# andrewcharlesjones/spatial-alignment

Measured on AMD Instinct MI355X. Metric: training steps/sec (ELBO fwd+bwd), 2-view N=10k M=200, 1/2/4/8 GPU, higher is better.
Workload: dtype f32 (fp64 warp layer, covariance whitening and M x M factorisations)

## Files before the change

### spatial_alignment_amd/csrc/qf_common.hpp

```cpp
#pragma once
#include <stdlib.h>

#include "common.hpp"

namespace gpsa {

typedef float f32x4_t __attribute__((ext_vector_type(4)));

typedef float f32x4 __attribute__((ext_vector_type(4)));
typedef float f32x2 __attribute__((ext_vector_type(2)));

enum { MODE_QUAD = 0, MODE_ACCUM = 1, MODE_STORE = 2 };

enum { PACK_SYM_UPPER = 1, PACK_KSTEP = 2, PACK_KSTEP_LAST = 4 };

typedef __attribute__((address_space(3))) void* lds_ptr_t;

__device__ __forceinline__ void glds16(const float* gsrc, unsigned lds_base) {
  unsigned keep;
  asm volatile(
      "s_mov_b32 %0, m0\n\ts_mov_b32 m0, %2\n\ts_nop 0\n\tglobal_load_lds_dwordx4 %1, off\n\ts_mov_b32 m0, %0"
      : "=&s"(keep)
      : "v"(gsrc), "s"(lds_base)
      : "memory");
}
__device__ __forceinline__ void dma_set_m0(unsigned lds_base) {
  asm volatile("s_mov_b32 m0, %0\n\ts_nop 0" ::"s"(lds_base) : "memory");
}
template <int IMM>
__device__ __forceinline__ void glds16_m0(const float* gsrc_minus_imm) {
  static_assert(IMM >= 0 && IMM < 4096, "immediate offset of a global instruction");
  asm volatile("global_load_lds_dwordx4 %0, off offset:%1" ::"v"(gsrc_minus_imm), "n"(IMM) : "memory");
}
template <int IMM>
__device__ __forceinline__ void glds4_m0(const float* gsrc_minus_imm) {
  static_assert(IMM >= 0 && IMM < 4096, "immediate offset of a global instruction");
  asm volatile("global_load_lds_dword %0, off offset:%1" ::"v"(gsrc_minus_imm), "n"(IMM) : "memory");
}
#define GPSA_DMA_DRAIN() asm volatile("s_waitcnt vmcnt(0)" ::: "memory")
#define GPSA_DMA_WAIT(N) asm volatile("s_waitcnt vmcnt(%0)" ::"n"(N) : "memory")
__device__ __forceinline__ unsigned lds_addr(const void* p) {
  return (unsigned)(unsigned long long)(lds_ptr_t)(p);
}

#define GPSA_PANEL_MAX_C (1LL << 26)
template <int MB, int NCT, bool QO, bool FULLT = false>
__device__ __forceinline__ void load_alpha_slab(const float* __restrict__ X, int M, long long C, long long cw, int j,
                                                int kq, float (&xb)[NCT][MB][4], bool (&okc)[NCT]) {
  const int Mm1 = M - 1;
  const unsigned Cu = (unsigned)C;
#pragma unroll
  for (int ct = 0; ct < NCT; ++ct) {
    const long long c = cw + ct * 16 + j;
    okc[ct] = c < C;
    const unsigned cl = (unsigned)(okc[ct] ? c : C - 1);
#pragma unroll
    for (int t = 0; t < MB; ++t)
#pragma unroll
      for (int r = 0; r < 4; ++r) {
        const int want = t * 16 + (QO ? r : r * 4);
        const int lane_row = QO ? kq * 4 : kq;
        if (FULLT && t < MB - 1) {
          xb[ct][t][r] = (X + (long long)want * C)[(unsigned)lane_row * Cu + cl];
        } else {
          const int bu = want < Mm1 ? want : Mm1;
          const int lp = lane_row < Mm1 - bu ? lane_row : Mm1 - bu;
          xb[ct][t][r] = (X + (long long)bu * C)[(unsigned)lp * Cu + cl];
        }
      }
  }
#pragma unroll
  for (int ct = 0; ct < NCT; ++ct)
#pragma unroll
    for (int t = 0; t < MB; ++t)
#pragma unroll
      for (int r = 0; r < 4; ++r)
        xb[ct][t][r] = (okc[ct] && t * 16 + (QO ? kq * 4 + r : r * 4 + kq) < M) ? xb[ct][t][r] : 0.f;
}
template <int MB, int NCT, int NR>
__device__ __forceinline__ void load_alpha_last(const float* __restrict__ X, int M, long long C, long long cw, int j,
                                                int kq, int nlive, float (&xl)[NCT][NR]) {
#pragma unroll
  for (int ct = 0; ct < NCT; ++ct) {
    const long long c = cw + ct * 16 + j;
    const bool ok = c < C;
    const float* __restrict__ Xc = X + (ok ? c : C - 1);
    float v[NR];
#pragma unroll
    for (int r = 0; r < NR; ++r) {
      const int row = (MB - 1) * 16 + r * 4 + kq;
      v[r] = Xc[(long long)(row < M ? row : M - 1) * C];
    }
#pragma unroll
    for (int r = 0; r < NR; ++r) xl[ct][r] = (r < nlive && ok && (MB - 1) * 16 + r * 4 + kq < M) ? v[r] : 0.f;
  }
}

struct TileOrder {
  long long tile0, tile1, nfull, n;
  int lo0, hi1, L, fp, lp;
  __device__ TileOrder(long long it0, long long it1, int L_) {
    L = L_;
    tile0 = it0 / L;
    tile1 = (it1 - 1) / L;
    lo0 = (int)(it0 - tile0 * L);
    hi1 = (int)(it1 - 1 - tile1 * L);
    if (tile0 == tile1) {
      fp = lp = 0;
      nfull = 0;
      n = 1;
    } else {
      fp = lo0 != 0;
      lp = hi1 != L - 1;
      nfull = (tile1 - lp) - (tile0 + fp) + 1;
      n = nfull + fp + lp;
    }
  }
  __device__ void get(long long step, long long& tile, int& a, int& b) const {
    if (tile0 == tile1) {
      tile = tile0; a = lo0; b = hi1;
    } else if (step < nfull) {
      tile = tile0 + fp + step; a = 0; b = L - 1;
    } else if (lp && step == nfull) {
      tile = tile1; a = 0; b = hi1;
    } else {
      tile = tile0; a = lo0; b = L - 1;
    }
  }
};

struct GramBigArgs {
  const float* alpha;
  const float* g;
  float* part;
  int M, L, nsplit, nblk;
  long long C, Cpad;
  int lb;
};
__global__ void pad_rows_kernel(const float* __restrict__ g, int L, long long C, long long Cpad,
                                float* __restrict__ gpad);
void gram_big_launch(dim3 grid, hipStream_t st, const GramBigArgs& a);
struct ProdBigArgs {
  const float* P;
  const float* X;
  float* W;
  int M, Mp, L;
  long long C;
};
__global__ void __launch_bounds__(256, 2) prod_big_kernel(ProdBigArgs a);
template <typename TO>
__global__ void __launch_bounds__(256) gram_big_reduce_kernel(const float* __restrict__ part, int M, int nsplit, TO* __restrict__ out);
static inline int big_remap_lb() { return 16; }

struct BigQuadArgs {
  const float* P;
  const float* X;
  float* v;
  float* W;
  int M, Mp, L;
  long long C;
  int lb;
};

struct BigAccumArgs {
  const float* P;
  const float* X;
  const float* g;
  float* out;
  int M, Mp, L, nrb, nsplit;
  long long C, ctiles;
  float scale;
};

__global__ void __launch_bounds__(256) big_accum_reduce_kernel(const float* __restrict__ part, int nsplit, long long n4, float* __restrict__ out);
static inline bool big_panel_ok(int M, long long C, int L, const void* alpha) {
  return M > 128 && (C & 3) == 0 && C >= 128 && cdiv(C, 128) * cdiv(M, 128) * 32 < 0x7fffffffLL && L <= 65535 &&
         (reinterpret_cast<uintptr_t>(alpha) & 15) == 0;
}
static inline int big_accum_nsplit(int M, long long C, int L) {
  const long long wgs = cdiv(M, 128) * cdiv(C, 128), slots = 2LL * num_cus();
  int best = 1;
  double beff = 0.0;
  for (int s = 1; s <= 4 && (s == 1 || L / s >= 8); ++s) {
    const double eff = (double)(wgs * s) / (double)(cdiv(wgs * s, slots) * slots);
    if (eff > beff) { beff = eff; best = s; }
    if (eff >= 0.9) break;
  }
  return best;
}
static inline long long big_accum_ws_bytes(int M, long long C, int L) {
  const int ns = big_accum_nsplit(M, C, L);
  return ns > 1 ? (long long)ns * M * C * 4 : 0;
}

template <typename TS>
__global__ void pad_k_kernel(const TS* __restrict__ src, int M, int Mp, long long n, float* __restrict__ dst);
template <typename TS>
__global__ void pad_k_tri_kernel(const TS* __restrict__ src, int M, int Mp, long long n, float* __restrict__ dst);
template <bool TRI, bool STORE, int NS>
__global__ void __launch_bounds__(256, 2) big_quad_kernel(BigQuadArgs a);
template <int NS>
__global__ void __launch_bounds__(256, 2) big_accum_kernel(BigAccumArgs a);
extern template __global__ void pad_k_kernel<float>(const float* __restrict__, int, int, long long, float* __restrict__);
extern template __global__ void pad_k_kernel<double>(const double* __restrict__, int, int, long long, float* __restrict__);
extern template __global__ void pad_k_tri_kernel<float>(const float* __restrict__, int, int, long long, float* __restrict__);
extern template __global__ void pad_k_tri_kernel<double>(const double* __restrict__, int, int, long long, float* __restrict__);
extern template __global__ void big_quad_kernel<true, false, 3>(BigQuadArgs);
extern template __global__ void big_quad_kernel<false, true, 3>(BigQuadArgs);
extern template __global__ void big_accum_kernel<3>(BigAccumArgs);
extern template __global__ void gram_big_reduce_kernel<float>(const float* __restrict__, int, int, float* __restrict__);

constexpr int panel_wgs_per_cu(int MB, int NCT) { return (MB * NCT >= 24) ? 1 : 2; }
constexpr int elbo_wgs_per_cu(int MB, int NCT) { return (MB * NCT >= 14) ? 1 : 2; }
#define GPSA_SHAPE_SECOND(MB, SECOND, ...) \
  if (mb == MB) return SECOND;

template <int MB, int NCT, int MODE, int RL>
__global__ void __launch_bounds__(256, panel_wgs_per_cu(MB, NCT)) panel_mfma_kernel(const float* __restrict__ Ppk, const float* __restrict__ X, const float* __restrict__ g, int M, long long C, int L, float* __restrict__ out, float* __restrict__ colsq, float out_scale, float* __restrict__ slab, float* __restrict__ keep);
#define GPSA_PANEL_SIG (const float* __restrict__ Ppk, const float* __restrict__ X, const float* __restrict__ g, int M, long long C, int L, float* __restrict__ out, float* __restrict__ colsq, float out_scale, float* __restrict__ slab, float* __restrict__ keep)
#define GPSA_PANEL_SHAPES(X, MODE) X(2, 4, MODE) X(4, 4, MODE) X(7, 4, MODE) X(13, 3, MODE) X(16, 2, MODE)
#define GPSA_PANEL_SHAPES_BIG(X, MODE) X(24, 1, MODE) X(32, 1, MODE)
#define GPSA_PANEL_EXTERN(MB, NCT, MODE)                                              \
  extern template __global__ void panel_mfma_kernel<MB, NCT, MODE, 2> GPSA_PANEL_SIG; \
  extern template __global__ void panel_mfma_kernel<MB, NCT, MODE, 4> GPSA_PANEL_SIG;
#define GPSA_PANEL_DEFINE(MB, NCT, MODE)                                       \
  template __global__ void panel_mfma_kernel<MB, NCT, MODE, 2> GPSA_PANEL_SIG; \
  template __global__ void panel_mfma_kernel<MB, NCT, MODE, 4> GPSA_PANEL_SIG;
GPSA_PANEL_SHAPES(GPSA_PANEL_EXTERN, MODE_QUAD)
GPSA_PANEL_SHAPES(GPSA_PANEL_EXTERN, MODE_STORE)
GPSA_PANEL_SHAPES(GPSA_PANEL_EXTERN, MODE_ACCUM)
GPSA_PANEL_SHAPES_BIG(GPSA_PANEL_EXTERN, MODE_ACCUM)
constexpr int panel_nct_for(int mb) {
  GPSA_PANEL_SHAPES(GPSA_SHAPE_SECOND, 0)
  GPSA_PANEL_SHAPES_BIG(GPSA_SHAPE_SECOND, 0)
  return 0;
}

struct ElboArgs {
  const float* Ppk;
  const float* X;
  int M;
  long long C;
  int L;
  const float* meanT;
  const double* q;
  const float* var_u;
  const float* eps;
  const float* Y;
  const float* noise_u;
  long long N;
  int S;
  float* g;
  float* dmeanT;
  float* FT;
  float* abar;
  float* slab;
  double* part;
  int nparts;
};

template <int MB, int NCT, int RL, bool FULLT = false, bool PAIRB = false>
__global__ void __launch_bounds__(256, elbo_wgs_per_cu(MB, NCT)) panel_elbo_kernel(ElboArgs a);
#define GPSA_ELBO_SHAPES(X) X(2, 4) X(4, 4) X(7, 4) X(13, 2) X(16, 2)
#define GPSA_ELBO_EXTERN(MB, NCT)                                          \
  extern template __global__ void panel_elbo_kernel<MB, NCT, 2>(ElboArgs); \
  extern template __global__ void panel_elbo_kernel<MB, NCT, 4>(ElboArgs);
#define GPSA_ELBO_DEFINE(MB, NCT)                                   \
  template __global__ void panel_elbo_kernel<MB, NCT, 2>(ElboArgs); \
  template __global__ void panel_elbo_kernel<MB, NCT, 4>(ElboArgs);
GPSA_ELBO_SHAPES(GPSA_ELBO_EXTERN)
constexpr int elbo_nct_for(int mb) {
  GPSA_ELBO_SHAPES(GPSA_SHAPE_SECOND)
  return 0;
}
extern template __global__ void panel_elbo_kernel<13, 2, 2, true, true>(ElboArgs);
extern template __global__ void panel_elbo_kernel<13, 2, 4, true, true>(ElboArgs);
template <int MB, int NCT, int RL, bool FULLT = false, bool PAIRB = false>
__global__ void __launch_bounds__(256, elbo_wgs_per_cu(MB, NCT)) panel_elbo_skip_kernel(ElboArgs a);
#define GPSA_ELBO_SKIP_EXTERN(MB, NCT)                                          \
  extern template __global__ void panel_elbo_skip_kernel<MB, NCT, 2>(ElboArgs); \
  extern template __global__ void panel_elbo_skip_kernel<MB, NCT, 4>(ElboArgs);
#define GPSA_ELBO_SKIP_DEFINE(MB, NCT)                                   \
  template __global__ void panel_elbo_skip_kernel<MB, NCT, 2>(ElboArgs); \
  template __global__ void panel_elbo_skip_kernel<MB, NCT, 4>(ElboArgs);
GPSA_ELBO_SHAPES(GPSA_ELBO_SKIP_EXTERN)
extern template __global__ void panel_elbo_skip_kernel<13, 2, 2, true, true>(ElboArgs);
extern template __global__ void panel_elbo_skip_kernel<13, 2, 4, true, true>(ElboArgs);
template <int MB, int NCT, int RL, bool FULLT = false, bool PAIRB = false>
__global__ void __launch_bounds__(256, elbo_wgs_per_cu(MB, NCT))
panel_elbo_pois_kernel(ElboArgs a, const float* __restrict__ log_offset, int skip);
#define GPSA_ELBO_POIS_EXTERN(MB, NCT)                                                              \
  extern template __global__ void panel_elbo_pois_kernel<MB, NCT, 2>(ElboArgs, const float*, int); \
  extern template __global__ void panel_elbo_pois_kernel<MB, NCT, 4>(ElboArgs, const float*, int);
#define GPSA_ELBO_POIS_DEFINE(MB, NCT)                                                       \
  template __global__ void panel_elbo_pois_kernel<MB, NCT, 2>(ElboArgs, const float*, int); \
  template __global__ void panel_elbo_pois_kernel<MB, NCT, 4>(ElboArgs, const float*, int);
GPSA_ELBO_SHAPES(GPSA_ELBO_POIS_EXTERN)
extern template __global__ void panel_elbo_pois_kernel<13, 2, 2, true, true>(ElboArgs, const float*, int);
extern template __global__ void panel_elbo_pois_kernel<13, 2, 4, true, true>(ElboArgs, const float*, int);

template <int MB, int NCT>
__global__ void __launch_bounds__(256, 1) panel_elbo_x3_kernel(ElboArgs a);
#define GPSA_ELBO_X3_SHAPES(X) X(2, 2) X(4, 2) X(7, 2) X(13, 1) X(16, 1)
#define GPSA_ELBO_X3_EXTERN(MB, NCT) extern template __global__ void panel_elbo_x3_kernel<MB, NCT>(ElboArgs);
#define GPSA_ELBO_X3_DEFINE(MB, NCT) template __global__ void panel_elbo_x3_kernel<MB, NCT>(ElboArgs);
GPSA_ELBO_X3_SHAPES(GPSA_ELBO_X3_EXTERN)
constexpr int elbo_x3_nct_for(int mb) {
  GPSA_ELBO_X3_SHAPES(GPSA_SHAPE_SECOND)
  return 0;
}
template <typename TS>
__global__ void __launch_bounds__(256) pack_x3_kernel(const TS* __restrict__ src, int M, int MB, int KB, int L,
                                                       unsigned short* __restrict__ dst, const float* __restrict__ drow);
extern template __global__ void pack_x3_kernel<float>(const float* __restrict__, int, int, int, int,
                                                      unsigned short* __restrict__, const float* __restrict__);
extern template __global__ void pack_x3_kernel<double>(const double* __restrict__, int, int, int, int,
                                                       unsigned short* __restrict__, const float* __restrict__);

template <int MB, int NCT, int RL>
__global__ void __launch_bounds__(256, panel_wgs_per_cu(MB, NCT)) quad_sym_mfma_kernel(const float* __restrict__ Ppk, const float* __restrict__ X, int M, long long C, int L, float* __restrict__ out);
#define GPSA_SYM_SIG (const float* __restrict__ Ppk, const float* __restrict__ X, int M, long long C, int L, float* __restrict__ out)
#define GPSA_SYM_SHAPES(X) X(2, 4) X(4, 4) X(7, 4) X(13, 3) X(16, 2) X(24, 1)
#define GPSA_SYM_EXTERN(MB, NCT)                                                 \
  extern template __global__ void quad_sym_mfma_kernel<MB, NCT, 2> GPSA_SYM_SIG; \
  extern template __global__ void quad_sym_mfma_kernel<MB, NCT, 4> GPSA_SYM_SIG;
#define GPSA_SYM_DEFINE(MB, NCT)                                          \
  template __global__ void quad_sym_mfma_kernel<MB, NCT, 2> GPSA_SYM_SIG; \
  template __global__ void quad_sym_mfma_kernel<MB, NCT, 4> GPSA_SYM_SIG;
GPSA_SYM_SHAPES(GPSA_SYM_EXTERN)

constexpr int GR_KC = 64;
template <int MB, bool ALIGNED, int NL>
__global__ void __launch_bounds__(256, (MB >= 13 || NL > 1) ? 1 : 2) gram_mfma_kernel(const float* __restrict__ alpha, const float* __restrict__ g, long long gstride, int M, long long C, int L, int nsplit, float* __restrict__ part, const float* __restrict__ dmean);
#define GPSA_GRAM_SIG (const float* __restrict__ alpha, const float* __restrict__ g, long long gstride, int M, long long C, int L, int nsplit, float* __restrict__ part, const float* __restrict__ dmean)
template <int MB>
struct GramPlan {
  static constexpr int NT = MB * (MB + 1) / 2;
  int cnt[4];
  int rr[4][NT], cc[4][NT];
  constexpr GramPlan() : cnt{}, rr{}, cc{} {
    const int cap = (NT + 3) / 4;
    for (int r = MB - 1; r >= 0; --r) {
      int best = -1;
      for (int w = 0; w < 4 && best < 0; ++w)
        if (cnt[w] + r + 1 <= cap) best = w;
      if (best < 0) {
        best = 0;
        for (int w = 1; w < 4; ++w)
          if (cnt[w] < cnt[best]) best = w;
      }
      for (int c = 0; c <= r; ++c) {
        rr[best][cnt[best]] = r;
        cc[best][cnt[best]] = c;
        ++cnt[best];
      }
    }
  }
  constexpr int max_cnt() const {
    int m = 0;
    for (int w = 0; w < 4; ++w) m = cnt[w] > m ? cnt[w] : m;
    return m;
  }
};

#define GPSA_GRAM_SHAPES(X) X(2, 2) X(4, 2) X(7, 2) X(13, 2) X(2, 1) X(4, 1) X(7, 1) X(13, 1) X(16, 1)
#define GPSA_GRAM_EXTERN(MB, NL)                                                \
  extern template __global__ void gram_mfma_kernel<MB, true, NL> GPSA_GRAM_SIG; \
  extern template __global__ void gram_mfma_kernel<MB, false, NL> GPSA_GRAM_SIG;
#define GPSA_GRAM_DEFINE(MB, NL)                                         \
  template __global__ void gram_mfma_kernel<MB, true, NL> GPSA_GRAM_SIG; \
  template __global__ void gram_mfma_kernel<MB, false, NL> GPSA_GRAM_SIG;
GPSA_GRAM_SHAPES(GPSA_GRAM_EXTERN)
constexpr int gram_max_nl(int mb) {
  GPSA_GRAM_SHAPES(GPSA_SHAPE_SECOND)
  return 0;
}
template <typename TO>
__global__ void gram_reduce_kernel(const float* __restrict__ part, int M, int MP, int L, int nsplit, TO* __restrict__ out,
                                   float* __restrict__ ddelta, float dbeta);
extern template __global__ void gram_reduce_kernel<float>(const float* __restrict__, int, int, int, int, float* __restrict__, float* __restrict__, float);
extern template __global__ void gram_reduce_kernel<double>(const float* __restrict__, int, int, int, int, double* __restrict__, float* __restrict__, float);

template <int MB>
__global__ void __launch_bounds__(256, 1) gram_x3_kernel(const unsigned short* __restrict__ img, const float* __restrict__ g,
                                                         const float* __restrict__ dmean, int M, long long C, int L,
                                                         int nsplit, float* __restrict__ part);
#define GPSA_GRAM_X3_SHAPES(X) X(2) X(4) X(7) X(13) X(16)
#define GPSA_GRAM_X3_EXTERN(MB)                                                                                          \
  extern template __global__ void gram_x3_kernel<MB>(const unsigned short* __restrict__, const float* __restrict__,       \
                                                     const float* __restrict__, int, long long, int, int, float* __restrict__);
GPSA_GRAM_X3_SHAPES(GPSA_GRAM_X3_EXTERN)
__global__ void __launch_bounds__(256) split_image_kernel(const float* __restrict__ X, int M, int MB, long long C, long long KBc,
                                                          unsigned short* __restrict__ dst);

}
```

### spatial_alignment_amd/csrc/qf_gram.hip

```cpp
#include "qf_common.hpp"

namespace gpsa {

__device__ __attribute__((aligned(16))) const float gram_zero16[4] = {0.f, 0.f, 0.f, 0.f};


constexpr int GR_G = 4;

template <int MB, int NKB, int W, int NS, int NL, typename STG>
__device__ __forceinline__ void gram_wave_chunk(const float* __restrict__ img,
                                                const float* __restrict__ gvec, int kq,
                                                f32x4 (&acc)[NL][NS + GR_G], STG&& stage, int drow, int lane15) {
  constexpr GramPlan<MB> P{};
  constexpr int N = P.cnt[W];
  constexpr int NGRP = (((NS + GR_G - 1) / GR_G) + 1) & ~1;
  constexpr int NPW_ = (MB * NKB + 3) / 4;
  static_assert(NKB == 4, "one K block per staging wave");
  auto frag = [&](int kb, int tile_row) {
    return *reinterpret_cast<const float4*>(img + kb * (NPW_ * 256) + tile_row * 256);
  };
  auto tile_of = [](int s) { return s < N ? s : N - 1; };
  auto new_row = [&](int s) { return s < N && (s == 0 || P.rr[W][s] != P.rr[W][s - 1]); };
  float4 araw[2][GR_G], fb[2][GR_G];
  float4 gk[NL], gn[NL], arow[NL];
#pragma unroll
  for (int q = 0; q < NL; ++q) {
    gn[q] = gk[q] = *reinterpret_cast<const float4*>(gvec + q * GR_KC + kq * 4);
    arow[q] = make_float4(0.f, 0.f, 0.f, 0.f);
  }
  constexpr bool OWNS_LAST = [] {
    constexpr GramPlan<MB> Q{};
    for (int s = 0; s < Q.cnt[W]; ++s)
      if (Q.rr[W][s] == MB - 1) return true;
    return false;
  }();
  const bool dsel = OWNS_LAST && drow >= 0 && lane15 == drow;
  float4 dk[OWNS_LAST ? NL : 1], dn[OWNS_LAST ? NL : 1];
  if (OWNS_LAST) {
#pragma unroll
    for (int q = 0; q < NL; ++q)
      dn[q] = dk[q] = drow >= 0 ? *reinterpret_cast<const float4*>(gvec + (NL + q) * GR_KC + kq * 4)
                                : make_float4(0.f, 0.f, 0.f, 0.f);
  }
#define GPSA_GR_FETCH(SLOT, KB, GP)                                                           \
  _Pragma("unroll") for (int u = 0; u < GR_G; ++u) {                                          \
    const int t__ = tile_of(GR_G * (GP) + u);                                                 \
    if (new_row(GR_G * (GP) + u)) araw[SLOT][u] = frag(KB, P.rr[W][t__]);                     \
    fb[SLOT][u] = frag(KB, P.cc[W][t__]);                                                     \
  }
  GPSA_GR_FETCH(0, 0, 0)
#pragma unroll 1
  for (int kb = 0; kb < NKB; ++kb) {
#pragma unroll
    for (int q = 0; q < NL; ++q) gk[q] = gn[q];
    if (OWNS_LAST) {
#pragma unroll
      for (int q = 0; q < NL; ++q) dk[q] = dn[q];
    }
#pragma unroll
    for (int gp = 0; gp < NGRP; ++gp) {
      const int cur = gp & 1, nxt = cur ^ 1;
      if (gp + 1 < NGRP) {
        GPSA_GR_FETCH(nxt, kb, gp + 1)
      } else if (kb + 1 < NKB) {
#pragma unroll
        for (int q = 0; q < NL; ++q)
          gn[q] = *reinterpret_cast<const float4*>(gvec + q * GR_KC + (kb + 1) * 16 + kq * 4);
        if (OWNS_LAST && drow >= 0) {
#pragma unroll
          for (int q = 0; q < NL; ++q)
            dn[q] = *reinterpret_cast<const float4*>(gvec + (NL + q) * GR_KC + (kb + 1) * 16 + kq * 4);
        }
        GPSA_GR_FETCH(nxt, kb + 1, 0)
      }
      __builtin_amdgcn_sched_barrier(0);
      if (gp < 5) stage(kb, gp);
      __builtin_amdgcn_sched_barrier(0);
      float4 a[NL][GR_G];
      int sl[GR_G];
#pragma unroll
      for (int u = 0; u < GR_G; ++u) {
        const int s_ = GR_G * gp + u;
        sl[u] = s_ < N ? s_ : NS + u;
#pragma unroll
        for (int q = 0; q < NL; ++q) {
          if (new_row(s_)) {
            const float4 r_ = araw[cur][u];
            arow[q] = make_float4(r_.x * gk[q].x, r_.y * gk[q].y, r_.z * gk[q].z, r_.w * gk[q].w);
            if (OWNS_LAST && P.rr[W][s_ < N ? s_ : N - 1] == MB - 1 && drow >= 0) {
              const float4 d_ = dk[q];
              arow[q] = make_float4(dsel ? d_.x : arow[q].x, dsel ? d_.y : arow[q].y, dsel ? d_.z : arow[q].z,
                                    dsel ? d_.w : arow[q].w);
            }
          }
          a[q][u] = arow[q];
        }
      }
#define GPSA_GR_MMA(F)                                                                          \
  _Pragma("unroll") for (int q = 0; q < NL; ++q)                                                \
    _Pragma("unroll") for (int u = 0; u < GR_G; ++u)                                            \
      if (GR_G * gp + u < N)                                                                    \
        acc[q][sl[u]] = __builtin_amdgcn_mfma_f32_16x16x4f32(a[q][u].F, fb[cur][u].F, acc[q][sl[u]], 0, 0, 0);
      GPSA_GR_MMA(x)
      GPSA_GR_MMA(y)
      GPSA_GR_MMA(z)
      GPSA_GR_MMA(w)
#undef GPSA_GR_MMA
      __builtin_amdgcn_sched_barrier(0);
    }
  }
#undef GPSA_GR_FETCH
}

template <int MB, int W, int NS>
__device__ __forceinline__ void gram_wave_store(const f32x4 (&acc)[NS + GR_G], float* __restrict__ P_, int j,
                                                int kq) {
  constexpr GramPlan<MB> P{};
  constexpr int MP = MB * 16;
#pragma unroll
  for (int s = 0; s < P.cnt[W]; ++s)
#pragma unroll
    for (int r = 0; r < 4; ++r)
      P_[(long long)(P.rr[W][s] * 16 + kq * 4 + r) * MP + P.cc[W][s] * 16 + j] = acc[s][r];
}

template <int MB, bool ALIGNED, int NL, int W>
__device__ __forceinline__ void gram_wave_run(const float* __restrict__ alpha, const float* __restrict__ g,
                                              long long gstride, int M, long long C, int L, int nsplit, float* __restrict__ part,
                                              float* __restrict__ sA_, float* __restrict__ sG_,
                                              const float* __restrict__ dmean) {
  constexpr int MP = MB * 16;
  constexpr GramPlan<MB> PLAN{};
  constexpr int NS = PLAN.max_cnt();
  constexpr int NKB = GR_KC / 16, NPIECE = MB * NKB;
  constexpr int NPW = (NPIECE + 3) / 4;
  constexpr int SA_STRIDE = NPW * 4 * 256, SG_STRIDE = 2 * NL * GR_KC;
  const int nstage = (dmean != nullptr ? 2 : 1) * NL * (GR_KC / 4);
  const int drow = dmean != nullptr ? M - 16 * (MB - 1) : -1;
  const int tid = threadIdx.x, lane = tid & 63;
  constexpr int w = W;
  const int j = lane & 15, kq = lane >> 4;
  const int l0 = blockIdx.x * NL, sp = blockIdx.y;
  const long long nch = (C + GR_KC - 1) / GR_KC;
  const long long ch0 = (long long)sp * nch / nsplit, ch1 = (long long)(sp + 1) * nch / nsplit;

  f32x4 acc[NL][NS + GR_G];
#pragma unroll
  for (int q = 0; q < NL; ++q)
#pragma unroll
    for (int s = 0; s < NS + GR_G; ++s) acc[q][s] = (f32x4){0.f, 0.f, 0.f, 0.f};

  auto gsrc = [&](int ln, long long col) -> const float* {
    const int which = ln / (NL * (GR_KC / 4)), lq = min(l0 + (ln / (GR_KC / 4)) % NL, L - 1);
    if (which == 1) return col >= C ? gram_zero16 : dmean + (long long)lq * C + col;
    return (gstride == C && col >= C) ? gram_zero16 : g + (long long)lq * gstride + col;
  };
#define GPSA_GR_STAGE(CH, BUF)                                                               \
  {                                                                                          \
    const long long cb__ = (long long)(CH) * GR_KC;                                          \
    if (ALIGNED) {                                                                           \
       \
      long long col = cb__ + w * 16 + kq * 4;                                                \
      col = col < C - 4 ? col : C - 4;                                                       \
      _Pragma("unroll") for (int pc = 0; pc < NPW; ++pc) {                                   \
        if ((pc & 3) == 0)                                                                   \
          dma_set_m0(__builtin_amdgcn_readfirstlane(lds_addr(sA_ + (BUF) * SA_STRIDE + (w * NPW + pc) * 256))); \
        int row = (pc < MB ? pc : 0) * 16 + j;                                               \
        row = row < M ? row : M - 1;                                                         \
        const float* gp__ = alpha + (long long)row * C + col;                                \
        if ((pc & 3) == 0) glds16_m0<0>(gp__);                                               \
        if ((pc & 3) == 1) glds16_m0<1024>(gp__ - 256);                                      \
        if ((pc & 3) == 2) glds16_m0<2048>(gp__ - 512);                                      \
        if ((pc & 3) == 3) glds16_m0<3072>(gp__ - 768);                                      \
      }                                                                                      \
      if (lane < nstage) {                                                                   \
        dma_set_m0(__builtin_amdgcn_readfirstlane(lds_addr(sG_ + (BUF) * SG_STRIDE)));       \
        glds16_m0<0>(gsrc(lane, cb__ + (lane % (GR_KC / 4)) * 4));                           \
      }                                                                                      \
    } else {                                                                                 \
      for (int e = tid; e < NPIECE * 256; e += 256) {                                        \
        const int piece = e >> 8, ln = (e >> 2) & 63, r = e & 3;                             \
        const int rb = piece / NKB, kb = piece % NKB;                                        \
        const int row = rb * 16 + (ln & 15);                                                 \
        const long long col = cb__ + kb * 16 + (ln >> 4) * 4 + r;                            \
        sA_[(BUF) * SA_STRIDE + (kb * NPW + rb) * 256 + (e & 255)] =                         \
            (row < M && col < C) ? alpha[(long long)row * C + col] : 0.f;                    \
      }                                                                                      \
      if (tid < NL * GR_KC)           \
        sG_[(BUF) * SG_STRIDE + tid] = g[(long long)min(l0 + tid / GR_KC, L - 1) * gstride + cb__ + tid % GR_KC]; \
    }                                                                                        \
  }

  if (ch1 > ch0) GPSA_GR_STAGE(ch0, 0)
  GPSA_DMA_DRAIN();
  __syncthreads();
  int buf = 0;
  for (long long ch = ch0; ch < ch1; ++ch) {
    const bool more = ch + 1 < ch1;
    constexpr int NGRP_ = (((NS + GR_G - 1) / GR_G) + 1) & ~1;
    constexpr bool SPREAD = ALIGNED && NGRP_ >= 5;
    if (more && !SPREAD) GPSA_GR_STAGE(ch + 1, buf ^ 1)
    const float* img = sA_ + buf * SA_STRIDE + lane * 4;
    long long ncol = (ch + 1) * GR_KC + w * 16 + kq * 4;
    ncol = ncol < C - 4 ? ncol : C - 4;
    const float* nsrc = alpha + ncol;
    float* nimg = sA_ + (buf ^ 1) * SA_STRIDE + w * NPW * 256;
    auto stage = [&](int kb, int gp) {
      if (!SPREAD || !more) return;
      if (gp < 4) {
        const int pc = kb * 4 + gp;
        if (pc < NPW) {
          if (gp == 0) dma_set_m0(__builtin_amdgcn_readfirstlane(lds_addr(nimg + kb * 4 * 256)));
          int row = pc * 16 + j;
          row = row < M ? row : M - 1;
          const float* gp__ = nsrc + (long long)row * C;
          if (gp == 0) glds16_m0<0>(gp__);
          if (gp == 1) glds16_m0<1024>(gp__ - 256);
          if (gp == 2) glds16_m0<2048>(gp__ - 512);
          if (gp == 3) glds16_m0<3072>(gp__ - 768);
        }
      } else if (kb == 0 && lane < nstage) {
        dma_set_m0(__builtin_amdgcn_readfirstlane(lds_addr(sG_ + (buf ^ 1) * SG_STRIDE)));
        glds16_m0<0>(gsrc(lane, (ch + 1) * GR_KC + (lane % (GR_KC / 4)) * 4));
      }
    };
    static_assert(NPW <= 16, "four pieces per K block of the chunk being multiplied");
    gram_wave_chunk<MB, NKB, W, NS, NL>(img, sG_ + buf * SG_STRIDE, kq, acc, stage, drow, lane & 15);
    GPSA_DMA_DRAIN();
    __syncthreads();
    buf ^= 1;
  }
  GPSA_DMA_DRAIN();
#undef GPSA_GR_STAGE
#pragma unroll
  for (int q = 0; q < NL; ++q) {
    if (l0 + q >= L) break;
    float* P = part + ((long long)(l0 + q) * nsplit + sp) * MP * MP;
    gram_wave_store<MB, W, NS>(acc[q], P, j, kq);
  }
}

template <int MB, bool ALIGNED, int NL>
__global__ void __launch_bounds__(256, (MB >= 13 || NL > 1) ? 1 : 2)
gram_mfma_kernel(const float* __restrict__ alpha, const float* __restrict__ g, long long gstride, int M,
                 long long C, int L, int nsplit, float* __restrict__ part, const float* __restrict__ dmean) {
  constexpr int NKB = GR_KC / 16, NPIECE = MB * NKB;
  constexpr int NPW = (NPIECE + 3) / 4;
  __shared__ __attribute__((aligned(16))) float sA[2][NPW * 4 * 256];
  __shared__ __attribute__((aligned(16))) float sG[2][2 * NL * GR_KC];
  const int w = __builtin_amdgcn_readfirstlane(threadIdx.x >> 6);
  switch (w) {
    case 0: gram_wave_run<MB, ALIGNED, NL, 0>(alpha, g, gstride, M, C, L, nsplit, part, &sA[0][0], &sG[0][0], dmean); break;
    case 1: gram_wave_run<MB, ALIGNED, NL, 1>(alpha, g, gstride, M, C, L, nsplit, part, &sA[0][0], &sG[0][0], dmean); break;
    case 2: gram_wave_run<MB, ALIGNED, NL, 2>(alpha, g, gstride, M, C, L, nsplit, part, &sA[0][0], &sG[0][0], dmean); break;
    default: gram_wave_run<MB, ALIGNED, NL, 3>(alpha, g, gstride, M, C, L, nsplit, part, &sA[0][0], &sG[0][0], dmean); break;
  }
}

template <typename TO>
__global__ void gram_reduce_kernel(const float* __restrict__ part, int M, int MP, int L, int nsplit,
                                   TO* __restrict__ out, float* __restrict__ ddelta, float dbeta) {
  const int jj = blockIdx.x * 32 + (threadIdx.x & 31);
  const int i = blockIdx.y * 8 + (threadIdx.x >> 5);
  const int l = blockIdx.z;
  if (ddelta != nullptr && i == M && jj < M) {
    const float* p = part + (long long)l * nsplit * MP * MP + (long long)M * MP + jj;
    const long long mm = (long long)MP * MP;
    double s = 0.0;
    for (int sp = 0; sp < nsplit; ++sp) s += (double)p[sp * mm];
    float* d = ddelta + (long long)jj * L + l;
    *d = dbeta != 0.f ? dbeta * *d + (float)s : (float)s;
    return;
  }
  if (i >= M || jj > i) return;
  const float* p = part + (long long)l * nsplit * MP * MP + (long long)i * MP + jj;
  const long long mm = (long long)MP * MP;
  TO s = TO(0), s1 = TO(0), s2 = TO(0), s3 = TO(0);
  int sp = 0;
  for (; sp + 3 < nsplit; sp += 4) {
    s += (TO)p[sp * mm];
    s1 += (TO)p[(sp + 1) * mm];
    s2 += (TO)p[(sp + 2) * mm];
    s3 += (TO)p[(sp + 3) * mm];
  }
  for (; sp < nsplit; ++sp) s += (TO)p[sp * mm];
  s = (s + s1) + (s2 + s3);
  TO* o = out + (long long)l * M * M;
  o[(long long)i * M + jj] = s;
  if (jj != i) o[(long long)jj * M + i] = s;
}


GPSA_GRAM_SHAPES(GPSA_GRAM_DEFINE)
template __global__ void gram_reduce_kernel<float>(const float* __restrict__, int, int, int, int, float* __restrict__, float* __restrict__, float);
template __global__ void gram_reduce_kernel<double>(const float* __restrict__, int, int, int, int, double* __restrict__, float* __restrict__, float);

}
```

Before: 151.5.

## Pair two outputs in the half-empty last tile row of the Gram MFMA kernel

When M leaves the last 16-row tile at most half full (M=200 gives 8 of 16 rows, MB=13), the two outputs (NL=2) now share one MFMA for each last-row tile. Lanes 8-15 carry the second output's weighted rows, which cuts the MFMA count in that row by half. The rebalanced wave plan uses 8-wide groups for the paired tiles. The mean-correction (d delta) row is moved out of the MFMA into packed v_pk_fma_f32 VALU accumulators with a cross-lane shuffle reduction. The cost is more template instantiations, register pressure and complex scheduling, with correctness guarded by compile-time plan validation.

```diff
diff --git a/spatial_alignment_amd/csrc/qf_common.hpp b/spatial_alignment_amd/csrc/qf_common.hpp
--- a/spatial_alignment_amd/csrc/qf_common.hpp
+++ b/spatial_alignment_amd/csrc/qf_common.hpp
@@ -333,26 +333,62 @@
 template <int MB, bool ALIGNED, int NL>
 __global__ void __launch_bounds__(256, (MB >= 13 || NL > 1) ? 1 : 2) gram_mfma_kernel(const float* __restrict__ alpha, const float* __restrict__ g, long long gstride, int M, long long C, int L, int nsplit, float* __restrict__ part, const float* __restrict__ dmean);
 #define GPSA_GRAM_SIG (const float* __restrict__ alpha, const float* __restrict__ g, long long gstride, int M, long long C, int L, int nsplit, float* __restrict__ part, const float* __restrict__ dmean)
-template <int MB>
+template <int MB, bool PAIR = false>
 struct GramPlan {
   static constexpr int NT = MB * (MB + 1) / 2;
   int cnt[4];
   int rr[4][NT], cc[4][NT];
-  constexpr GramPlan() : cnt{}, rr{}, cc{} {
-    const int cap = (NT + 3) / 4;
-    for (int r = MB - 1; r >= 0; --r) {
+  int ng[4];
+  int gs[4][NT + 2], gn[4][NT + 2];
+  int nr[4], ri[4][NT];
+  static constexpr int GCAP = PAIR ? 8 : 4;
+  static constexpr int cost(int r) { return PAIR ? (r == MB - 1 ? MB : 2 * (r + 1)) : r + 1; }
+  constexpr GramPlan() : cnt{}, rr{}, cc{}, ng{}, gs{}, gn{}, nr{}, ri{} {
+    int total = 0;
+    for (int r = 0; r < MB; ++r) total += cost(r);
+    const int cap = (total + 3) / 4;
+    int load[4] = {0, 0, 0, 0}, rows[4][MB] = {}, nrows[4] = {0, 0, 0, 0};
+    bool used[MB] = {};
+    for (int k = 0; k < MB; ++k) {
+      int r = -1;
+      for (int q = MB - 1; q >= 0; --q)
+        if (!used[q] && (r < 0 || cost(q) > cost(r))) r = q;
+      used[r] = true;
       int best = -1;
       for (int w = 0; w < 4 && best < 0; ++w)
-        if (cnt[w] + r + 1 <= cap) best = w;
+        if (load[w] + cost(r) <= cap) best = w;
       if (best < 0) {
         best = 0;
         for (int w = 1; w < 4; ++w)
-          if (cnt[w] < cnt[best]) best = w;
+          if (load[w] < load[best]) best = w;
       }
-      for (int c = 0; c <= r; ++c) {
-        rr[best][cnt[best]] = r;
-        cc[best][cnt[best]] = c;
-        ++cnt[best];
+      rows[best][nrows[best]++] = r;
+      load[best] += cost(r);
+    }
+    for (int w = 0; w < 4; ++w) {
+      for (int pass = PAIR ? 0 : 1; pass < 2; ++pass)
+        for (int k = 0; k < nrows[w]; ++k) {
+          const int r = rows[w][k];
+          if (PAIR && (r == MB - 1) != (pass == 0)) continue;
+          for (int c = 0; c <= r; ++c) {
+            rr[w][cnt[w]] = r;
+            cc[w][cnt[w]] = c;
+            ++cnt[w];
+          }
+        }
+      nr[w] = nrows[w];
+      for (int s = 1; s < cnt[w]; ++s) ri[w][s] = ri[w][s - 1] + (rr[w][s] != rr[w][s - 1] ? 1 : 0);
+      int np = 0;
+      for (int s = 0; s < cnt[w]; ++s) np += (PAIR && rr[w][s] == MB - 1) ? 1 : 0;
+      const int rawp = (np + 7) / 8, rawn = (cnt[w] - np + 3) / 4;
+      ng[w] = (rawp + rawn + 1) & ~1;
+      int at = 0;
+      for (int g = 0; g < ng[w]; ++g) {
+        gs[w][g] = at;
+        if (g < rawp) gn[w][g] = np / rawp + (g < np % rawp ? 1 : 0);
+        else if (g < rawp + rawn) gn[w][g] = (cnt[w] - np) / rawn + (g - rawp < (cnt[w] - np) % rawn ? 1 : 0);
+        else gn[w][g] = 0;
+        at += gn[w][g];
       }
     }
   }
@@ -361,7 +397,57 @@
     for (int w = 0; w < 4; ++w) m = cnt[w] > m ? cnt[w] : m;
     return m;
   }
-};
+  constexpr int min_ng() const {
+    int m = ng[0];
+    for (int w = 1; w < 4; ++w) m = ng[w] < m ? ng[w] : m;
+    return m;
+  }
+  constexpr int slots(int w, int nl) const {
+    int n = 0;
+    for (int s = 0; s < cnt[w]; ++s) n += (PAIR && rr[w][s] == MB - 1) ? 1 : nl;
+    return n;
+  }
+  constexpr int max_slots(int nl) const {
+    int m = 0;
+    for (int w = 0; w < 4; ++w) m = slots(w, nl) > m ? slots(w, nl) : m;
+    return m;
+  }
+  constexpr int sum_slots(int nl) const { return slots(0, nl) + slots(1, nl) + slots(2, nl) + slots(3, nl); }
+  constexpr bool valid() const {
+    for (int r = 0; r < MB; ++r)
+      for (int c = 0; c <= r; ++c) {
+        int n = 0;
+        for (int w = 0; w < 4; ++w)
+          for (int s = 0; s < cnt[w]; ++s) n += (rr[w][s] == r && cc[w][s] == c) ? 1 : 0;
+        if (n != 1) return false;
+      }
+    for (int w = 0; w < 4; ++w) {
+      int at = 0;
+      for (int g = 0; g < ng[w]; ++g) {
+        if (gs[w][g] != at || gn[w][g] < 0 || gn[w][g] > GCAP) return false;
+        at += gn[w][g];
+      }
+      if (at != cnt[w] || (ng[w] & 1)) return false;
+    }
+    return true;
+  }
+};
+static_assert(GramPlan<2>{}.valid() && GramPlan<4>{}.valid() && GramPlan<7>{}.valid() && GramPlan<13>{}.valid() &&
+                  GramPlan<16>{}.valid(),
+              "every lower tile is owned exactly once");
+static_assert(GramPlan<2, true>{}.valid() && GramPlan<4, true>{}.valid() && GramPlan<7, true>{}.valid() &&
+                  GramPlan<13, true>{}.valid(),
+              "every lower tile is owned exactly once (paired last tile row)");
+static_assert(GramPlan<13>{}.sum_slots(2) == 182 && GramPlan<13>{}.max_slots(2) == 46, "MB = 13, two outputs: 23 tiles");
+static_assert(GramPlan<13>{}.cnt[0] == 23 && GramPlan<13>{}.cnt[1] == 23 && GramPlan<13>{}.cnt[2] == 23 &&
+                  GramPlan<13>{}.cnt[3] == 22,
+              "the unpaired deal is the one the kernel has always run");
+static_assert(GramPlan<13, true>{}.sum_slots(2) == 169 && GramPlan<13, true>{}.max_slots(2) == 43,
+              "MB = 13, paired last tile row: 2 x 78 + 13 slots, at most 43 on a wave");
+static_assert(GramPlan<13, true>{}.min_ng() >= 5, "the next chunk's LDS-DMA rides in groups 0-4 of every wave");
+static_assert(GramPlan<13, true>{}.ng[0] == 6 && GramPlan<13, true>{}.ng[1] == 6 && GramPlan<13, true>{}.ng[2] == 6 &&
+                  GramPlan<13, true>{}.ng[3] == 6,
+              "six groups per K block on every wave, as in the unpaired schedule");
 
 #define GPSA_GRAM_SHAPES(X) X(2, 2) X(4, 2) X(7, 2) X(13, 2) X(2, 1) X(4, 1) X(7, 1) X(13, 1) X(16, 1)
 #define GPSA_GRAM_EXTERN(MB, NL)                                                \
diff --git a/spatial_alignment_amd/csrc/qf_gram.hip b/spatial_alignment_amd/csrc/qf_gram.hip
--- a/spatial_alignment_amd/csrc/qf_gram.hip
+++ b/spatial_alignment_amd/csrc/qf_gram.hip
@@ -7,21 +7,31 @@
 
 constexpr int GR_G = 4;
 
-template <int MB, int NKB, int W, int NS, int NL, typename STG>
+template <int MB, int NKB, int W, int NS, int NL, bool PAIR, bool DD, int NR, typename STG>
 __device__ __forceinline__ void gram_wave_chunk(const float* __restrict__ img,
                                                 const float* __restrict__ gvec, int kq,
-                                                f32x4 (&acc)[NL][NS + GR_G], STG&& stage, int drow, int lane15) {
-  constexpr GramPlan<MB> P{};
+                                                f32x4 (&acc)[NL][NS + GR_G], f32x2 (&dacc)[NR], STG&& stage, int drow,
+                                                int lane15) {
+  constexpr GramPlan<MB, PAIR> P{};
   constexpr int N = P.cnt[W];
-  constexpr int NGRP = (((NS + GR_G - 1) / GR_G) + 1) & ~1;
+  constexpr int GC = P.GCAP;
+  constexpr int NGRP = PAIR ? P.ng[W] : (((NS + GR_G - 1) / GR_G) + 1) & ~1;
+  static_assert(!PAIR || NL == 2, "two outputs share the last tile row");
   constexpr int NPW_ = (MB * NKB + 3) / 4;
   static_assert(NKB == 4, "one K block per staging wave");
   auto frag = [&](int kb, int tile_row) {
     return *reinterpret_cast<const float4*>(img + kb * (NPW_ * 256) + tile_row * 256);
   };
+  const float* imgp = img - (PAIR && lane15 >= 8 ? 32 : 0);
+  auto fragp = [&](int kb, int tile_row) {
+    return *reinterpret_cast<const float4*>(imgp + kb * (NPW_ * 256) + tile_row * 256);
+  };
   auto tile_of = [](int s) { return s < N ? s : N - 1; };
   auto new_row = [&](int s) { return s < N && (s == 0 || P.rr[W][s] != P.rr[W][s - 1]); };
-  float4 araw[2][GR_G], fb[2][GR_G];
+  auto slot = [&](int gp, int u) { return PAIR ? P.gs[W][gp] + u : GR_G * gp + u; };
+  auto live = [&](int gp, int u) { return PAIR ? u < P.gn[W][gp] : GR_G * gp + u < N; };
+  auto paired = [&](int s) { return PAIR && s < N && P.rr[W][s] == MB - 1; };
+  float4 araw[2][GC], fb[2][GC];
   float4 gk[NL], gn[NL], arow[NL];
 #pragma unroll
   for (int q = 0; q < NL; ++q) {
@@ -29,23 +39,28 @@
     arow[q] = make_float4(0.f, 0.f, 0.f, 0.f);
   }
   constexpr bool OWNS_LAST = [] {
-    constexpr GramPlan<MB> Q{};
+    constexpr GramPlan<MB, PAIR> Q{};
     for (int s = 0; s < Q.cnt[W]; ++s)
       if (Q.rr[W][s] == MB - 1) return true;
     return false;
   }();
-  const bool dsel = OWNS_LAST && drow >= 0 && lane15 == drow;
-  float4 dk[OWNS_LAST ? NL : 1], dn[OWNS_LAST ? NL : 1];
-  if (OWNS_LAST) {
+  const bool dsel = !PAIR && OWNS_LAST && drow >= 0 && lane15 == drow;
+  constexpr bool DK = PAIR ? DD && N > 0 : OWNS_LAST;
+  static_assert(PAIR || !DD, "DD: the vector-ALU d delta of the paired schedule");
+  float4 dk[DK ? NL : 1], dn[DK ? NL : 1];
+  float4 gsel = make_float4(0.f, 0.f, 0.f, 0.f);
+  if (DK) {
 #pragma unroll
     for (int q = 0; q < NL; ++q)
       dn[q] = dk[q] = drow >= 0 ? *reinterpret_cast<const float4*>(gvec + (NL + q) * GR_KC + kq * 4)
                                 : make_float4(0.f, 0.f, 0.f, 0.f);
   }
 #define GPSA_GR_FETCH(SLOT, KB, GP)                                                           \
-  _Pragma("unroll") for (int u = 0; u < GR_G; ++u) {                                          \
-    const int t__ = tile_of(GR_G * (GP) + u);                                                 \
-    if (new_row(GR_G * (GP) + u)) araw[SLOT][u] = frag(KB, P.rr[W][t__]);                     \
+  _Pragma("unroll") for (int u = 0; u < GC; ++u) {                                            \
+    if (PAIR && !live(GP, u)) continue;                                                       \
+    const int t__ = tile_of(slot(GP, u));                                                     \
+    if (new_row(slot(GP, u)))                                                                 \
+      araw[SLOT][u] = paired(slot(GP, u)) ? fragp(KB, P.rr[W][t__]) : frag(KB, P.rr[W][t__]); \
     fb[SLOT][u] = frag(KB, P.cc[W][t__]);                                                     \
   }
   GPSA_GR_FETCH(0, 0, 0)
@@ -53,9 +68,21 @@
   for (int kb = 0; kb < NKB; ++kb) {
 #pragma unroll
     for (int q = 0; q < NL; ++q) gk[q] = gn[q];
-    if (OWNS_LAST) {
+    if (DK) {
 #pragma unroll
       for (int q = 0; q < NL; ++q) dk[q] = dn[q];
+    }
+    f32x2 dkp[4];
+    if (DD && DK) {
+      dkp[0] = (f32x2){dk[0].x, dk[NL - 1].x};
+      dkp[1] = (f32x2){dk[0].y, dk[NL - 1].y};
+      dkp[2] = (f32x2){dk[0].z, dk[NL - 1].z};
+      dkp[3] = (f32x2){dk[0].w, dk[NL - 1].w};
+    }
+    if (PAIR && OWNS_LAST) {
+      const bool hi = lane15 >= 8;
+      gsel = make_float4(hi ? gk[NL - 1].x : gk[0].x, hi ? gk[NL - 1].y : gk[0].y, hi ? gk[NL - 1].z : gk[0].z,
+                         hi ? gk[NL - 1].w : gk[0].w);
     }
 #pragma unroll
     for (int gp = 0; gp < NGRP; ++gp) {
@@ -66,7 +93,7 @@
 #pragma unroll
         for (int q = 0; q < NL; ++q)
           gn[q] = *reinterpret_cast<const float4*>(gvec + q * GR_KC + (kb + 1) * 16 + kq * 4);
-        if (OWNS_LAST && drow >= 0) {
+        if (DK && drow >= 0) {
 #pragma unroll
           for (int q = 0; q < NL; ++q)
             dn[q] = *reinterpret_cast<const float4*>(gvec + (NL + q) * GR_KC + (kb + 1) * 16 + kq * 4);
@@ -76,18 +103,20 @@
       __builtin_amdgcn_sched_barrier(0);
       if (gp < 5) stage(kb, gp);
       __builtin_amdgcn_sched_barrier(0);
-      float4 a[NL][GR_G];
-      int sl[GR_G];
-#pragma unroll
-      for (int u = 0; u < GR_G; ++u) {
-        const int s_ = GR_G * gp + u;
-        sl[u] = s_ < N ? s_ : NS + u;
+      float4 a[NL][GC];
+      int sl[GC];
+#pragma unroll
+      for (int u = 0; u < GC; ++u) {
+        const int s_ = slot(gp, u);
+        sl[u] = (PAIR ? live(gp, u) : s_ < N) ? s_ : (PAIR ? 0 : NS + u);
+        if (PAIR && !live(gp, u)) continue;
 #pragma unroll
         for (int q = 0; q < NL; ++q) {
           if (new_row(s_)) {
             const float4 r_ = araw[cur][u];
-            arow[q] = make_float4(r_.x * gk[q].x, r_.y * gk[q].y, r_.z * gk[q].z, r_.w * gk[q].w);
-            if (OWNS_LAST && P.rr[W][s_ < N ? s_ : N - 1] == MB - 1 && drow >= 0) {
+            const float4 g_ = paired(s_) ? gsel : gk[q];
+            arow[q] = make_float4(r_.x * g_.x, r_.y * g_.y, r_.z * g_.z, r_.w * g_.w);
+            if (!PAIR && OWNS_LAST && P.rr[W][s_ < N ? s_ : N - 1] == MB - 1 && drow >= 0) {
               const float4 d_ = dk[q];
               arow[q] = make_float4(dsel ? d_.x : arow[q].x, dsel ? d_.y : arow[q].y, dsel ? d_.z : arow[q].z,
                                     dsel ? d_.w : arow[q].w);
@@ -98,13 +127,29 @@
       }
 #define GPSA_GR_MMA(F)                                                                          \
   _Pragma("unroll") for (int q = 0; q < NL; ++q)                                                \
-    _Pragma("unroll") for (int u = 0; u < GR_G; ++u)                                            \
-      if (GR_G * gp + u < N)                                                                    \
+    _Pragma("unroll") for (int u = 0; u < GC; ++u)                                              \
+      if (live(gp, u) && !(q > 0 && paired(slot(gp, u))))                                       \
         acc[q][sl[u]] = __builtin_amdgcn_mfma_f32_16x16x4f32(a[q][u].F, fb[cur][u].F, acc[q][sl[u]], 0, 0, 0);
+#define GPSA_GR_DD(HALF, SEL, KF)                                                                       \
+  if (DD) {                                                                                             \
+    _Pragma("unroll") for (int u = 0; u < GC; ++u)                                                      \
+      if (live(gp, u) && new_row(slot(gp, u))) {                                                        \
+        const f32x2 a2__ = HALF == 0 ? (f32x2){araw[cur][u].x, araw[cur][u].y}                          \
+                                     : (f32x2){araw[cur][u].z, araw[cur][u].w};                         \
+        asm volatile("v_pk_fma_f32 %0, %1, %2, %0 " SEL                                                 \
+                     : "+v"(dacc[P.ri[W][slot(gp, u)]])                                                 \
+                     : "v"(a2__), "v"(dkp[KF]));                                                        \
+      }                                                                                                 \
+  }
       GPSA_GR_MMA(x)
+      GPSA_GR_DD(0, "op_sel_hi:[0,1,1]", 0)
       GPSA_GR_MMA(y)
+      GPSA_GR_DD(0, "op_sel:[1,0,0]", 1)
       GPSA_GR_MMA(z)
+      GPSA_GR_DD(1, "op_sel_hi:[0,1,1]", 2)
       GPSA_GR_MMA(w)
+      GPSA_GR_DD(1, "op_sel:[1,0,0]", 3)
+#undef GPSA_GR_DD
 #undef GPSA_GR_MMA
       __builtin_amdgcn_sched_barrier(0);
     }
@@ -112,26 +157,53 @@
 #undef GPSA_GR_FETCH
 }
 
-template <int MB, int W, int NS>
-__device__ __forceinline__ void gram_wave_store(const f32x4 (&acc)[NS + GR_G], float* __restrict__ P_, int j,
-                                                int kq) {
-  constexpr GramPlan<MB> P{};
+template <int MB, int W, int NS, int NL, bool PAIR>
+__device__ __forceinline__ void gram_wave_store(const f32x4 (&acc)[NL][NS + GR_G], int q, float* __restrict__ P_, int M,
+                                                int j, int kq) {
+  constexpr GramPlan<MB, PAIR> P{};
   constexpr int MP = MB * 16;
 #pragma unroll
-  for (int s = 0; s < P.cnt[W]; ++s)
+  for (int s = 0; s < P.cnt[W]; ++s) {
+    if (PAIR && P.rr[W][s] == MB - 1) {
+      if ((kq >> 1) != q) continue;
+#pragma unroll
+      for (int r = 0; r < 4; ++r) {
+        const int row = (MB - 1) * 16 + (kq & 1) * 4 + r;
+        if (row < M) P_[(long long)row * MP + P.cc[W][s] * 16 + j] = acc[0][s][r];
+      }
+      continue;
+    }
 #pragma unroll
     for (int r = 0; r < 4; ++r)
-      P_[(long long)(P.rr[W][s] * 16 + kq * 4 + r) * MP + P.cc[W][s] * 16 + j] = acc[s][r];
-}
-
-template <int MB, bool ALIGNED, int NL, int W>
+      P_[(long long)(P.rr[W][s] * 16 + kq * 4 + r) * MP + P.cc[W][s] * 16 + j] = acc[q][s][r];
+  }
+}
+
+template <int MB, int W, int NR>
+__device__ __forceinline__ void gram_wave_ddelta(const f32x2 (&dacc)[NR], int q, float* __restrict__ P_, int M, int j,
+                                                 int kq) {
+  constexpr GramPlan<MB, true> P{};
+  constexpr int MP = MB * 16;
+#pragma unroll
+  for (int s = 0; s < P.cnt[W]; ++s) {
+    if (s > 0 && P.rr[W][s] == P.rr[W][s - 1]) continue;
+    float v = q == 0 ? dacc[P.ri[W][s]].x : dacc[P.ri[W][s]].y;
+    v += __shfl_xor(v, 16);
+    v += __shfl_xor(v, 32);
+    const int col = P.rr[W][s] * 16 + j;
+    if (kq == 0 && col < M) P_[(long long)M * MP + col] = v;
+  }
+}
+
+template <int MB, bool ALIGNED, int NL, int W, bool PAIR, bool DD = false>
 __device__ __forceinline__ void gram_wave_run(const float* __restrict__ alpha, const float* __restrict__ g,
                                               long long gstride, int M, long long C, int L, int nsplit, float* __restrict__ part,
                                               float* __restrict__ sA_, float* __restrict__ sG_,
                                               const float* __restrict__ dmean) {
   constexpr int MP = MB * 16;
-  constexpr GramPlan<MB> PLAN{};
+  constexpr GramPlan<MB, PAIR> PLAN{};
   constexpr int NS = PLAN.max_cnt();
+  constexpr int NR = DD && PLAN.nr[W] > 0 ? PLAN.nr[W] : 1;
   constexpr int NKB = GR_KC / 16, NPIECE = MB * NKB;
   constexpr int NPW = (NPIECE + 3) / 4;
   constexpr int SA_STRIDE = NPW * 4 * 256, SG_STRIDE = 2 * NL * GR_KC;
@@ -149,6 +221,9 @@
   for (int q = 0; q < NL; ++q)
 #pragma unroll
     for (int s = 0; s < NS + GR_G; ++s) acc[q][s] = (f32x4){0.f, 0.f, 0.f, 0.f};
+  f32x2 dacc[NR];
+#pragma unroll
+  for (int i = 0; i < NR; ++i) dacc[i] = (f32x2){0.f, 0.f};
 
   auto gsrc = [&](int ln, long long col) -> const float* {
     const int which = ln / (NL * (GR_KC / 4)), lq = min(l0 + (ln / (GR_KC / 4)) % NL, L - 1);
@@ -197,7 +272,7 @@
   int buf = 0;
   for (long long ch = ch0; ch < ch1; ++ch) {
     const bool more = ch + 1 < ch1;
-    constexpr int NGRP_ = (((NS + GR_G - 1) / GR_G) + 1) & ~1;
+    constexpr int NGRP_ = PAIR ? PLAN.min_ng() : (((NS + GR_G - 1) / GR_G) + 1) & ~1;
     constexpr bool SPREAD = ALIGNED && NGRP_ >= 5;
     if (more && !SPREAD) GPSA_GR_STAGE(ch + 1, buf ^ 1)
     const float* img = sA_ + buf * SA_STRIDE + lane * 4;
@@ -225,7 +300,7 @@
       }
     };
     static_assert(NPW <= 16, "four pieces per K block of the chunk being multiplied");
-    gram_wave_chunk<MB, NKB, W, NS, NL>(img, sG_ + buf * SG_STRIDE, kq, acc, stage, drow, lane & 15);
+    gram_wave_chunk<MB, NKB, W, NS, NL, PAIR, DD, NR>(img, sG_ + buf * SG_STRIDE, kq, acc, dacc, stage, drow, lane & 15);
     GPSA_DMA_DRAIN();
     __syncthreads();
     buf ^= 1;
@@ -236,7 +311,8 @@
   for (int q = 0; q < NL; ++q) {
     if (l0 + q >= L) break;
     float* P = part + ((long long)(l0 + q) * nsplit + sp) * MP * MP;
-    gram_wave_store<MB, W, NS>(acc[q], P, j, kq);
+    gram_wave_store<MB, W, NS, NL, PAIR>(acc, q, P, M, j, kq);
+    if constexpr (DD) gram_wave_ddelta<MB, W, NR>(dacc, q, P, M, j, kq);
   }
 }
 
@@ -249,11 +325,33 @@
   __shared__ __attribute__((aligned(16))) float sA[2][NPW * 4 * 256];
   __shared__ __attribute__((aligned(16))) float sG[2][2 * NL * GR_KC];
   const int w = __builtin_amdgcn_readfirstlane(threadIdx.x >> 6);
+  if constexpr (NL == 2) {
+    if (M > 16 * (MB - 1) && M <= 16 * (MB - 1) + 8) {
+      if constexpr (ALIGNED) {
+        if (dmean != nullptr) {
+          switch (w) {
+            case 0: gram_wave_run<MB, ALIGNED, NL, 0, true, true>(alpha, g, gstride, M, C, L, nsplit, part, &sA[0][0], &sG[0][0], dmean); break;
+            case 1: gram_wave_run<MB, ALIGNED, NL, 1, true, true>(alpha, g, gstride, M, C, L, nsplit, part, &sA[0][0], &sG[0][0], dmean); break;
+            case 2: gram_wave_run<MB, ALIGNED, NL, 2, true, true>(alpha, g, gstride, M, C, L, nsplit, part, &sA[0][0], &sG[0][0], dmean); break;
+            default: gram_wave_run<MB, ALIGNED, NL, 3, true, true>(alpha, g, gstride, M, C, L, nsplit, part, &sA[0][0], &sG[0][0], dmean); break;
+          }
+          return;
+        }
+      }
+      switch (w) {
+        case 0: gram_wave_run<MB, ALIGNED, NL, 0, true>(alpha, g, gstride, M, C, L, nsplit, part, &sA[0][0], &sG[0][0], nullptr); break;
+        case 1: gram_wave_run<MB, ALIGNED, NL, 1, true>(alpha, g, gstride, M, C, L, nsplit, part, &sA[0][0], &sG[0][0], nullptr); break;
+        case 2: gram_wave_run<MB, ALIGNED, NL, 2, true>(alpha, g, gstride, M, C, L, nsplit, part, &sA[0][0], &sG[0][0], nullptr); break;
+        default: gram_wave_run<MB, ALIGNED, NL, 3, true>(alpha, g, gstride, M, C, L, nsplit, part, &sA[0][0], &sG[0][0], nullptr); break;
+      }
+      return;
+    }
+  }
   switch (w) {
-    case 0: gram_wave_run<MB, ALIGNED, NL, 0>(alpha, g, gstride, M, C, L, nsplit, part, &sA[0][0], &sG[0][0], dmean); break;
-    case 1: gram_wave_run<MB, ALIGNED, NL, 1>(alpha, g, gstride, M, C, L, nsplit, part, &sA[0][0], &sG[0][0], dmean); break;
-    case 2: gram_wave_run<MB, ALIGNED, NL, 2>(alpha, g, gstride, M, C, L, nsplit, part, &sA[0][0], &sG[0][0], dmean); break;
-    default: gram_wave_run<MB, ALIGNED, NL, 3>(alpha, g, gstride, M, C, L, nsplit, part, &sA[0][0], &sG[0][0], dmean); break;
+    case 0: gram_wave_run<MB, ALIGNED, NL, 0, false>(alpha, g, gstride, M, C, L, nsplit, part, &sA[0][0], &sG[0][0], dmean); break;
+    case 1: gram_wave_run<MB, ALIGNED, NL, 1, false>(alpha, g, gstride, M, C, L, nsplit, part, &sA[0][0], &sG[0][0], dmean); break;
+    case 2: gram_wave_run<MB, ALIGNED, NL, 2, false>(alpha, g, gstride, M, C, L, nsplit, part, &sA[0][0], &sG[0][0], dmean); break;
+    default: gram_wave_run<MB, ALIGNED, NL, 3, false>(alpha, g, gstride, M, C, L, nsplit, part, &sA[0][0], &sG[0][0], dmean); break;
   }
 }
 
```

After: 152.9 (median of 6 runs). About the same (+0.9%).
